# CVLAB-Unibo/Keypoint-Learning

Hardware: NVIDIA B200
Metric: points scored/sec (search+normals+features+RF+NMS) (higher is better)
Workload: dtype f32

## Files before the change

### keypoint_learning_b200/csrc/capi.cu

```cuda
#include <algorithm>
#include <cmath>
#include <cstdio>
#include <cstdlib>
#include <cstring>
#include <numeric>
#include "kpl_internal.h"

namespace kpl {
int pack_forest(const HostForestArrays& in, std::vector<PackedNode>& nodes, std::vector<int32_t>& roots, int& max_depth, int& max_var, std::string& err);
cudaError_t launch_all_flags(kpl_ctx* c, int64_t n);
}
using namespace kpl;

#define KPL_CUDA(call)                                                                              \
    do {                                                                                            \
        cudaError_t e__ = (call);                                                                   \
        if (e__ != cudaSuccess) {                                                                   \
            char b__[512];                                                                          \
            snprintf(b__, sizeof b__, "%s:%d: %s -> %s", __FILE__, __LINE__, #call, cudaGetErrorString(e__)); \
            ctx->err = b__;                                                                         \
            return e__ == cudaErrorMemoryAllocation ? KPL_E_NOMEM : KPL_E_CUDA;                     \
        }                                                                                           \
    } while (0)

static int fail(kpl_ctx* ctx, int code, const std::string& msg)
{
    ctx->err = msg;
    return code;
}

static float dec_float(uint32_t u)
{
    uint32_t b = (u & 0x80000000u) ? (u & 0x7FFFFFFFu) : ~u;
    float f;
    memcpy(&f, &b, 4);
    return f;
}

template <typename T>
static void release(DevBuf<T>& b) { if (b.p) cudaFree(b.p); b.p = nullptr; b.cap = 0; }

extern "C" {

const char* kpl_version(void) { return "kpl-b200 0.1 (sm_100a)"; }

int kpl_device_count(void)
{
    int count = 0, usable = 0;
    if (cudaGetDeviceCount(&count) != cudaSuccess) { (void)cudaGetLastError(); return 0; }
    for (int d = 0; d < count; ++d) {
        cudaDeviceProp prop;
        if (cudaGetDeviceProperties(&prop, d) == cudaSuccess && prop.major == 10) usable++;
    }
    return usable;
}

int kpl_params_default(kpl_params* p)
{
    if (!p) return KPL_E_INVALID;
    memset(p, 0, sizeof *p);
    p->radius_features = 20.f;
    p->radius_nms = 4.f;
    p->threshold = (double)0.85f;
    p->n_annulus = 5;
    p->n_bins = 10;
    p->non_maxima = 1;
    p->draws_remove = 0;
    p->draws_threshold = 0.f;
    p->normals_mode = KPL_NORMALS_KNN;
    p->k_normals = 10;
    p->flip_normals = 0;
    p->cells_per_radius = 4;
    p->grid_forced = 0;
    p->slab_interior_lo = p->slab_interior_hi = 0;
    p->slab_guard_cells = 0;
    p->slab_owned_lo = p->slab_owned_hi = 0;
    p->uniform_sampling_centre = 0;
    p->eigen32_normalize = 0;
    p->report_fragile = 0;
    return KPL_OK;
}

int kpl_create(int device, kpl_ctx** out)
{
    if (!out) return KPL_E_INVALID;
    *out = nullptr;
    int count = 0;
    if (cudaGetDeviceCount(&count) != cudaSuccess || count <= 0 || device < 0 || device >= count) return KPL_E_CUDA;
    cudaDeviceProp prop;
    if (cudaGetDeviceProperties(&prop, device) != cudaSuccess) return KPL_E_CUDA;
    if (prop.major != 10) return KPL_E_CUDA;
    if (cudaSetDevice(device) != cudaSuccess) return KPL_E_CUDA;
    kpl_ctx* ctx = new (std::nothrow) kpl_ctx();
    if (!ctx) return KPL_E_NOMEM;
    ctx->device = device;
    kpl_params_default(&ctx->params);
    memset(&ctx->timings, 0, sizeof ctx->timings);
    memset(&ctx->stats, 0, sizeof ctx->stats);
    bool ok = cudaStreamCreateWithFlags(&ctx->own_stream, cudaStreamNonBlocking) == cudaSuccess;
    ctx->stream = ctx->own_stream;
    for (int i = 0; ok && i < 8; ++i) ok = cudaEventCreate(&ctx->ev[i]) == cudaSuccess;
    ok = ok && cudaMalloc((void**)&ctx->d_bbox, 8 * sizeof(uint32_t)) == cudaSuccess;
    ok = ok && ensure(ctx->counters, kpl_ctx::NCOUNTERS) == cudaSuccess;
    if (!ok) { kpl_destroy(ctx); return KPL_E_CUDA; }
    *out = ctx;
    return KPL_OK;
}

void kpl_destroy(kpl_ctx* ctx)
{
    if (!ctx) return;
    cudaSetDevice(ctx->device);
    if (ctx->own_stream) cudaStreamSynchronize(ctx->own_stream);
    release(ctx->in_xyz); release(ctx->in_nrm); release(ctx->in_role); release(ctx->s_role);
    release(ctx->key_a); release(ctx->key_b); release(ctx->idx_a); release(ctx->idx_b); release(ctx->cub_tmp);
    release(ctx->row_warps_n); release(ctx->row_offset_n); release(ctx->fragile); release(ctx->views); release(ctx->layer_view);
    release(ctx->view_offsets); release(ctx->qlist);
    release(ctx->cell_start); release(ctx->work_n); release(ctx->ckey_a); release(ctx->ckey_b); release(ctx->qorder_a); release(ctx->qorder_all); release(ctx->warp_starts_n); release(ctx->qorder_role); release(ctx->warp_starts_role);
    release(ctx->warp_order); release(ctx->s_pos); release(ctx->s_nrm); release(ctx->feat);
    release(ctx->s_score); release(ctx->score); release(ctx->flag); release(ctx->s_state); release(ctx->kp_idx);
    release(ctx->scratch_f); release(ctx->scratch_i); release(ctx->counters);
    if (ctx->d_bbox) cudaFree(ctx->d_bbox);
    if (ctx->forest.d_nodes) cudaFree(ctx->forest.d_nodes);
    if (ctx->forest.d_roots) cudaFree(ctx->forest.d_roots);
    for (int i = 0; i < 8; ++i) if (ctx->ev[i]) cudaEventDestroy(ctx->ev[i]);
    if (ctx->own_stream) cudaStreamDestroy(ctx->own_stream);
    delete ctx;
}

const char* kpl_last_error(const kpl_ctx* ctx) { return ctx ? ctx->err.c_str() : "null context"; }

int kpl_set_stream(kpl_ctx* ctx, void* s)
{
    if (!ctx) return KPL_E_INVALID;
    ctx->stream = s ? (cudaStream_t)s : ctx->own_stream;
    return KPL_OK;
}

int kpl_set_keep_intermediates(kpl_ctx* ctx, int on)
{
    if (!ctx) return KPL_E_INVALID;
    ctx->keep_intermediates = on != 0;
    return KPL_OK;
}

int kpl_set_params(kpl_ctx* ctx, const kpl_params* p)
{
    if (!ctx || !p) return KPL_E_INVALID;
    if (!(p->radius_features > 0.f) || !std::isfinite(p->radius_features)) return fail(ctx, KPL_E_INVALID, "radius_features must be > 0");
    if (p->radius_nms < 0.f || !std::isfinite(p->radius_nms)) return fail(ctx, KPL_E_INVALID, "radius_nms must be >= 0");
    if (p->n_annulus < 1 || p->n_bins < 1 || (int64_t)p->n_annulus * p->n_bins > 1022) return fail(ctx, KPL_E_INVALID, "annuli*bins must be in [1,1022]");
    if (p->normals_mode < 0 || p->normals_mode > 2) return fail(ctx, KPL_E_INVALID, "bad normals_mode");
    if (p->k_normals < 1 || p->k_normals > 64) return fail(ctx, KPL_E_INVALID, "k_normals must be in [1,64]");
    if (p->cells_per_radius < 1 || p->cells_per_radius > 16) return fail(ctx, KPL_E_INVALID, "cells_per_radius must be in [1,16]");
    ctx->params = *p;
    return KPL_OK;
}

int kpl_get_params(const kpl_ctx* ctx, kpl_params* p)
{
    if (!ctx || !p) return KPL_E_INVALID;
    *p = ctx->params;
    return KPL_OK;
}

static int install_forest(kpl_ctx* ctx, const HostForestArrays& H)
{
    std::vector<PackedNode> nodes;
    std::vector<int32_t> roots;
    int max_depth = 0, max_var = -1;
    std::string err;
    int rc = pack_forest(H, nodes, roots, max_depth, max_var, err);
    if (rc) return fail(ctx, rc, err);
    if (roots.empty()) return fail(ctx, KPL_E_FOREST, "forest has no trees");
    KPL_CUDA(cudaSetDevice(ctx->device));
    Forest& F = ctx->forest;
    if (F.d_nodes) cudaFree(F.d_nodes);
    if (F.d_roots) cudaFree(F.d_roots);
    F.d_nodes = nullptr; F.d_roots = nullptr; F.ntrees = 0;
    KPL_CUDA(cudaMalloc((void**)&F.d_nodes, nodes.size() * sizeof(PackedNode)));
    KPL_CUDA(cudaMalloc((void**)&F.d_roots, roots.size() * sizeof(int32_t)));
    KPL_CUDA(cudaMemcpy(F.d_nodes, nodes.data(), nodes.size() * sizeof(PackedNode), cudaMemcpyHostToDevice));
    KPL_CUDA(cudaMemcpy(F.d_roots, roots.data(), roots.size() * sizeof(int32_t), cudaMemcpyHostToDevice));
    F.ntrees = (int32_t)roots.size(); F.nnodes = (int32_t)H.var.size(); F.var_count = H.var_count; F.max_depth = max_depth; F.max_var = max_var;
    F.roots = roots;
    return KPL_OK;
}

int kpl_load_forest(kpl_ctx* ctx, const char* path)
{
    if (!ctx || !path) return KPL_E_INVALID;
    HostForestArrays H;
    std::string err;
    int rc = parse_forest_yaml(path, H, err);
    if (rc) return fail(ctx, rc, err);
    return install_forest(ctx, H);
}

int kpl_set_forest(kpl_ctx* ctx, int32_t ntrees, int32_t nnodes, const int32_t* roots, const int32_t* var, const float* thr,
                   const int32_t* left, const int32_t* right, const float* value, int32_t var_count)
{
    if (!ctx || ntrees < 1 || nnodes < 1 || !roots || !var || !thr || !left || !right || !value) return KPL_E_INVALID;
    HostForestArrays H;
    H.roots.assign(roots, roots + ntrees); H.var.assign(var, var + nnodes); H.thr.assign(thr, thr + nnodes);
    H.left.assign(left, left + nnodes); H.right.assign(right, right + nnodes); H.value.assign(value, value + nnodes);
    H.var_count = var_count;
    return install_forest(ctx, H);
}

int kpl_forest_info(const kpl_ctx* ctx, int32_t* ntrees, int32_t* nnodes, int32_t* var_count, int32_t* max_depth)
{
    if (!ctx) return KPL_E_INVALID;
    if (ntrees) *ntrees = ctx->forest.ntrees;
    if (nnodes) *nnodes = ctx->forest.nnodes;
    if (var_count) *var_count = ctx->forest.var_count;
    if (max_depth) *max_depth = ctx->forest.max_depth;
    return KPL_OK;
}

}

static const double CELL_PAD = 1.0 + 9.5367431640625e-07;
static const double REACH_PAD = 1.0 + 4.76837158203125e-07;

double kpl::canonical_cell(const kpl_params& P) { return (double)P.radius_features * CELL_PAD / (double)P.cells_per_radius; }
int32_t kpl::grid_dim(double lo, double hi, double cell) { return (int32_t)std::min(2147483000.0, std::floor((hi - lo) / cell) + 1.0); }
int kpl::grid_reach(double radius, double cell) { return (int)std::floor(radius * REACH_PAD / cell) + 1; }

static void clear_batch(GridDesc& g)
{
    g.views = nullptr; g.layer_view = nullptr; g.view_offsets = nullptr; g.nviews = 0;
    g.interior_lo = g.interior_hi = 0; g.guard_cells = 0;
    g.forced = 0;
}

static int finish_grid(kpl_ctx* ctx, int64_t n)
{
    GridDesc& g = ctx->grid;
    const kpl_params& P = ctx->params;
    double ncells = 1.0;
    for (int a = 0; a < 3; ++a) {
        if (g.dim[a] < 1) return fail(ctx, KPL_E_GRID, "bad grid dimensions");
        ncells *= (double)g.dim[a];
    }
    if (ncells > 2147483646.0) return fail(ctx, KPL_E_GRID, "uniform grid would exceed 2^31-2 cells: cloud too sparse for radius_features/cells_per_radius");
    g.ncells = (int64_t)ncells;
    g.reach_feat = grid_reach(P.radius_features, g.cell);
    g.reach_nms = grid_reach(P.radius_nms, g.cell);
    ctx->stats.grid_cells = g.ncells;
    for (int a = 0; a < 3; ++a) { ctx->stats.grid_dims[a] = g.dim[a]; ctx->stats.grid_origin[a] = g.org[a]; }
    ctx->stats.grid_cell = g.cell;
    ctx->last_n = n;
    return KPL_OK;
}

int kpl::prepare_grid(kpl_ctx* ctx, const float4* d_xyz, const float4* d_nrm, const uint8_t* d_role, int64_t n, const ForcedGrid* forced, double cell_override)
{
    GridDesc& g = ctx->grid;
    clear_batch(g);
    g.cell = cell_override > 0.0 ? cell_override : canonical_cell(ctx->params);
    if (forced) {
        KPL_CUDA(launch_bbox_init(ctx));
        for (int a = 0; a < 3; ++a) { g.org[a] = forced->origin[a]; g.dim[a] = forced->dims[a]; g.off[a] = forced->offset[a]; }
        g.interior_lo = forced->interior_lo; g.interior_hi = forced->interior_hi; g.guard_cells = forced->guard_cells;
        g.forced = 1;
    } else {
        KPL_CUDA(launch_bbox(ctx, d_xyz, n, ctx->d_bbox));
        uint32_t hb[8];
        KPL_CUDA(cudaMemcpyAsync(hb, ctx->d_bbox, sizeof hb, cudaMemcpyDeviceToHost, ctx->stream));
        KPL_CUDA(cudaStreamSynchronize(ctx->stream));
        ctx->syncs++;
        if (hb[6]) return fail(ctx, KPL_E_NONFINITE, "input cloud holds non-finite points");
        for (int a = 0; a < 3; ++a) {
            const double lo = (double)dec_float(hb[a]), hi = (double)dec_float(hb[3 + a]);
            g.off[a] = 0; g.org[a] = lo;
            g.dim[a] = grid_dim(lo, hi, g.cell);
        }
    }
    int rc = finish_grid(ctx, n);
    if (rc) return rc;
    ctx->cur_xyz = d_xyz;
    ctx->cur_nrm = d_nrm;
    KPL_CUDA(build_grid(ctx, d_xyz, d_nrm, d_role, n));
    return KPL_OK;
}

static int prepare_params_grid(kpl_ctx* ctx, const float4* d_xyz, const float4* d_nrm, const uint8_t* d_role, int64_t n)
{
    const kpl_params& P = ctx->params;
    if (!P.grid_forced) return prepare_grid(ctx, d_xyz, d_nrm, d_role, n, nullptr);
    ForcedGrid f;
    for (int a = 0; a < 3; ++a) { f.origin[a] = P.grid_origin[a]; f.dims[a] = P.grid_dims[a]; f.offset[a] = P.grid_offset[a]; }
    f.interior_lo = P.slab_interior_lo; f.interior_hi = P.slab_interior_hi; f.guard_cells = P.slab_guard_cells;
    return prepare_grid(ctx, d_xyz, d_nrm, d_role, n, &f);
}

static int prepare_grid_batch(kpl_ctx* ctx, const float4* d_xyz, const float4* d_nrm, int64_t n, const int64_t* h_offsets, int nviews)
{
    const kpl_params& P = ctx->params;
    GridDesc& g = ctx->grid;
    clear_batch(g);
    g.cell = canonical_cell(P);
    KPL_CUDA(ensure(ctx->view_offsets, (size_t)nviews + 1));
    KPL_CUDA(ensure(ctx->views, (size_t)nviews));
    KPL_CUDA(ensure(ctx->scratch_i, (size_t)nviews * 8 + 16));
    KPL_CUDA(cudaMemcpyAsync(ctx->view_offsets.p, h_offsets, ((size_t)nviews + 1) * sizeof(int64_t), cudaMemcpyHostToDevice, ctx->stream));
    KPL_CUDA(launch_bbox_init(ctx));
    uint32_t* d_boxes = (uint32_t*)ctx->scratch_i.p;
    KPL_CUDA(launch_bbox_views(ctx, d_xyz, n, ctx->view_offsets.p, nviews, d_boxes));
    std::vector<uint32_t> hb((size_t)nviews * 8);
    KPL_CUDA(cudaMemcpyAsync(hb.data(), d_boxes, hb.size() * sizeof(uint32_t), cudaMemcpyDeviceToHost, ctx->stream));
    KPL_CUDA(cudaStreamSynchronize(ctx->stream));
    ctx->syncs++;
    const int pad = std::max(std::max(grid_reach(P.radius_features, g.cell), grid_reach(P.radius_nms, g.cell)), 1);
    std::vector<ViewDesc> hv((size_t)nviews);
    int64_t z = 0;
    int dimx = 1, dimy = 1;
    for (int v = 0; v < nviews; ++v) {
        const uint32_t* b = hb.data() + (size_t)v * 8;
        if (b[6]) return fail(ctx, KPL_E_NONFINITE, "a view of the batch holds non-finite points");
        int d[3];
        for (int a = 0; a < 3; ++a) {
            const double lo = (double)dec_float(b[a]), hi = (double)dec_float(b[3 + a]);
            hv[(size_t)v].org[a] = lo;
            d[a] = grid_dim(lo, hi, g.cell);
        }
        dimx = std::max(dimx, d[0]); dimy = std::max(dimy, d[1]);
        hv[(size_t)v].zoff = (int32_t)z; hv[(size_t)v].dimz = d[2];
        z += (int64_t)d[2] + pad;
        if (z > 2147483000ll) return fail(ctx, KPL_E_GRID, "the stacked grid of the batch exceeds 2^31 layers");
    }
    g.dim[0] = dimx; g.dim[1] = dimy; g.dim[2] = (int32_t)(z - pad);
    for (int a = 0; a < 3; ++a) { g.off[a] = 0; g.org[a] = hv[0].org[a]; }
    int rc = finish_grid(ctx, n);
    if (rc) return rc;
    std::vector<int32_t> layer((size_t)g.dim[2], -1);
    for (int v = 0; v < nviews; ++v)
        for (int l = 0; l < hv[(size_t)v].dimz; ++l) layer[(size_t)hv[(size_t)v].zoff + l] = v;
    KPL_CUDA(ensure(ctx->layer_view, layer.size()));
    KPL_CUDA(cudaMemcpyAsync(ctx->views.p, hv.data(), hv.size() * sizeof(ViewDesc), cudaMemcpyHostToDevice, ctx->stream));
    KPL_CUDA(cudaMemcpyAsync(ctx->layer_view.p, layer.data(), layer.size() * sizeof(int32_t), cudaMemcpyHostToDevice, ctx->stream));
    KPL_CUDA(cudaStreamSynchronize(ctx->stream));
    ctx->syncs++;
    g.views = ctx->views.p; g.layer_view = ctx->layer_view.p; g.view_offsets = ctx->view_offsets.p; g.nviews = nviews;
    ctx->cur_xyz = d_xyz;
    ctx->cur_nrm = d_nrm;
    KPL_CUDA(build_grid(ctx, d_xyz, d_nrm, nullptr, n));
    return KPL_OK;
}

static int prepare_lists(kpl_ctx* ctx, bool normals_given, bool want_features, bool use_role)
{
    const kpl_params& P = ctx->params;
    int span_n = -1;
    bool curve_normals = false;
    if (!normals_given) {
        if (P.normals_mode == KPL_NORMALS_KNN) curve_normals = normals_knn_uses_work_list(P);
        else if (P.normals_mode == KPL_NORMALS_RADIUS) span_n = P.cells_per_radius;
    }
    const int64_t slots = 148 * 28;
    const int64_t longest_first_below = ctx->last_n * 32 < (int64_t)120e6 ? 24 * slots : 0;
    KPL_CUDA(build_lists(ctx, ctx->last_n, span_n, curve_normals, want_features, use_role, longest_first_below));
    return KPL_OK;
}

static int prepare_normals(kpl_ctx* ctx, bool given, int64_t n)
{
    const kpl_params& P = ctx->params;
    if (!given) {
        if (P.normals_mode == KPL_NORMALS_KNN) KPL_CUDA(launch_normals_knn(ctx, n));
        else if (P.normals_mode == KPL_NORMALS_RADIUS) KPL_CUDA(launch_normals_radius(ctx, n));
        else return fail(ctx, KPL_E_SIZE_MISMATCH, "normals_mode is GIVEN but no normals were passed");
        if (P.flip_normals) KPL_CUDA(launch_flip_normals(ctx, n));
    }
    ctx->last_has_normals = true;
    return KPL_OK;
}

void kpl::detect_reset(kpl_ctx* ctx)
{
    (void)cudaGetLastError();
    ctx->launches = 0;
    ctx->syncs = 0;
    ctx->err.clear();
    ctx->last_has_normals = ctx->last_has_features = ctx->last_has_fragile = false;
    memset(&ctx->timings, 0, sizeof ctx->timings);
    memset(&ctx->stats, 0, sizeof ctx->stats);
    ctx->stats.n_views = 1;
}

namespace kpl {

int detect_check(kpl_ctx* ctx, int64_t n, bool with_role)
{
    const kpl_params& P = ctx->params;
    if (n < 0 || n > 2147483000ll) return fail(ctx, KPL_E_INVALID, "point count out of range");
    if (ctx->forest.ntrees < 1) return fail(ctx, KPL_E_FOREST, "no forest loaded");
    if (P.draws_remove && P.non_maxima && with_role)
        return fail(ctx, KPL_E_UNSUPPORTED, "draws-remove NMS walks the whole cloud in index order (hpp:233-250): not available with a role array; use the kpl_shard_* entry points");
    const int F = P.n_annulus * P.n_bins;
    if (ctx->forest.var_count > 0 && ctx->forest.var_count != F) return fail(ctx, KPL_E_VARCOUNT, "annuli*bins does not match the forest's var_count");
    if (ctx->forest.max_var >= F) return fail(ctx, KPL_E_VARCOUNT, "the forest splits on a variable index >= annuli*bins");
    return KPL_OK;
}

int detect_score_phase(kpl_ctx* ctx, bool normals_given, bool use_role, int64_t n)
{
    const kpl_params& P = ctx->params;
    const int F = P.n_annulus * P.n_bins;
    int rc = prepare_lists(ctx, normals_given, true, use_role);
    if (rc) return rc;
    KPL_CUDA(cudaEventRecord(ctx->ev[1], ctx->stream));
    rc = prepare_normals(ctx, normals_given, n);
    if (rc) return rc;
    KPL_CUDA(launch_check_normals(ctx, n, use_role));
    KPL_CUDA(cudaEventRecord(ctx->ev[2], ctx->stream));
    bool fuse = true;
#ifdef KPL_EXPERIMENTS
    fuse = getenv("KPL_NO_FUSE") == nullptr;
#endif
    const bool rows = ctx->keep_intermediates || !fuse;
    KPL_CUDA(launch_features(ctx, n, use_role, fuse, rows));
    ctx->last_has_features = rows; ctx->last_F = F;
// ... 527 lines not shown
```

### keypoint_learning_b200/csrc/kpl_internal.h

```cpp
#pragma once
#include <cuda_runtime.h>
#include <stdint.h>
#include <string>
#include <vector>
#include "../../include/kpl.h"

namespace kpl {

struct ViewDesc {
    double org[3];
    int32_t zoff, dimz;
};
struct GridDesc {
    double org[3];
    double cell;
    int32_t dim[3];
    int32_t off[3];
    int32_t reach_feat;
    int32_t reach_nms;
    int64_t ncells;
    const ViewDesc* views;
    const int32_t* layer_view;
    const int64_t* view_offsets;
    int32_t nviews;
    int32_t interior_lo, interior_hi;
    int32_t guard_cells;
    int32_t forced;
};

struct ForcedGrid {
    double origin[3];
    int32_t dims[3], offset[3];
    int32_t interior_lo, interior_hi, guard_cells;
};

struct __align__(8) PackedNode {
    float thr;
    uint32_t packed;
};
static constexpr uint32_t KPL_LEAF_VAR = 1023u;

struct Forest {
    int32_t ntrees = 0, nnodes = 0, var_count = 0, max_depth = 0;
    int32_t max_var = -1;
    std::vector<int32_t> roots;
    PackedNode* d_nodes = nullptr;
    int32_t* d_roots = nullptr;
};

template <typename T>
struct DevBuf {
    T* p = nullptr;
    size_t cap = 0;
};

struct HostForestArrays {
    std::vector<int32_t> roots, var, left, right;
    std::vector<float> thr, value;
    int32_t var_count = 0;
};

int parse_forest_yaml(const char* path, HostForestArrays& out, std::string& err);

}

struct kpl_ctx {
    int device = 0;
    cudaStream_t own_stream = nullptr;
    cudaStream_t stream = nullptr;
    kpl_params params;
    kpl::Forest forest;
    kpl::GridDesc grid;
    kpl_timings timings;
    kpl_stats stats;
    std::string err;
    int launches = 0;

    kpl::DevBuf<float4> in_xyz, in_nrm;
    kpl::DevBuf<uint8_t> in_role, s_role;
    kpl::DevBuf<uint32_t> key_a, key_b, idx_a, idx_b;
    kpl::DevBuf<uint8_t> cub_tmp;
    kpl::DevBuf<int32_t> cell_start;
    kpl::DevBuf<int32_t> row_warps_n, row_offset_n;
    int nwarps_norm = 0, nwarps_feat = 0;
    kpl::DevBuf<int2> work_n;
    kpl::DevBuf<uint64_t> ckey_a, ckey_b;
    kpl::DevBuf<int32_t> qorder_a, qorder_all, warp_starts_n, qorder_role, warp_starts_role;
    const int32_t* qorder_f = nullptr;
    const int32_t* warp_starts_f = nullptr;
    kpl::DevBuf<uint32_t> warp_order;
    bool have_warp_order = false;
    kpl::DevBuf<float4> s_pos, s_nrm;
    kpl::DevBuf<float> feat;
    kpl::DevBuf<float> s_score, score;
    kpl::DevBuf<uint8_t> flag;
    kpl::DevBuf<uint8_t> fragile;
    kpl::DevBuf<kpl::ViewDesc> views;
    kpl::DevBuf<int32_t> layer_view;
    kpl::DevBuf<int64_t> view_offsets;
    kpl::DevBuf<int32_t> qlist;
    kpl::DevBuf<uint8_t> s_state;
    kpl::DevBuf<int32_t> kp_idx;
    kpl::DevBuf<float> scratch_f;
    kpl::DevBuf<int32_t> scratch_i;
    kpl::DevBuf<unsigned long long> counters;
    static constexpr int NCOUNTERS = 16;
    int syncs = 0;
    const float4* cur_xyz = nullptr;
    const float4* cur_nrm = nullptr;
    float* d_bbox = nullptr;
    int64_t last_n = 0;
    int last_F = 0;
    bool last_has_normals = false, last_has_features = false, last_has_fragile = false;
    bool fast_math = false;
    bool keep_intermediates = false;
    cudaEvent_t ev[8] = {nullptr, nullptr, nullptr, nullptr, nullptr, nullptr, nullptr, nullptr};
};

namespace kpl {

cudaError_t launch_bbox(kpl_ctx* c, const float4* xyz, int64_t n, float* d_bbox );
cudaError_t build_grid(kpl_ctx* c, const float4* xyz, const float4* nrm_or_null, const uint8_t* role_or_null, int64_t n);
cudaError_t launch_normals_knn(kpl_ctx* c, int64_t n);
cudaError_t launch_normals_radius(kpl_ctx* c, int64_t n);
cudaError_t launch_flip_normals(kpl_ctx* c, int64_t n);
cudaError_t launch_check_normals(kpl_ctx* c, int64_t n, bool use_role);
bool normals_knn_uses_work_list(const kpl_params& P);
cudaError_t launch_bbox_init(kpl_ctx* c);
cudaError_t launch_gather_keypoints(kpl_ctx* c, const float4* d_xyz, const int32_t* d_kp_idx, int64_t nkp, float4* d_out);
cudaError_t launch_normals_integral_image(kpl_ctx* c, const float4* d_xyz, int W, int H, float smoothing_size, float4* d_out);
cudaError_t build_lists(kpl_ctx* c, int64_t n, int span_n, bool curve_normals, bool want_features, bool use_role, int64_t longest_first_below);
cudaError_t launch_count_occupied_cells(kpl_ctx* c, int64_t n, unsigned long long* d_out);
cudaError_t build_query_list(kpl_ctx* c, int64_t n, const int32_t* d_indices, int64_t m);
cudaError_t launch_scatter_rows(kpl_ctx* c, const float* d_rows, int64_t m, int width, float* d_out);
cudaError_t launch_view_ranges(kpl_ctx* c, int64_t n, int32_t* d_kp_idx, const int64_t* d_view_offsets, int nviews, int64_t* d_kp_offsets);
cudaError_t launch_bbox_views(kpl_ctx* c, const float4* xyz, int64_t n, const int64_t* d_view_offsets, int nviews, uint32_t* d_bbox);
cudaError_t launch_features(kpl_ctx* c, int64_t n, bool use_role, bool fuse_forest, bool store_rows, const int32_t* d_qlist = nullptr, int64_t m_list = 0);
#ifdef KPL_EXPERIMENTS
cudaError_t launch_forest(kpl_ctx* c, int64_t n, bool use_role);
#endif
cudaError_t launch_nms(kpl_ctx* c, int64_t n, bool use_role);
cudaError_t launch_nms_draws(kpl_ctx* c, int64_t n, bool use_role);
cudaError_t launch_nms_draws_classify(kpl_ctx* c, int64_t n, bool use_role);
cudaError_t launch_nms_draws_round(kpl_ctx* c, int64_t n, bool use_role, const int32_t* gidx);
cudaError_t launch_nms_draws_flags(kpl_ctx* c, int64_t n, bool use_role);
inline int nms_round_cap(int64_t n) { return (int)(n < (1 << 20) ? n : (1 << 20)); }
cudaError_t launch_compact(kpl_ctx* c, int64_t n, int32_t* d_kp_idx_out);

cudaError_t uniform_sample(kpl_ctx* c, const float4* xyz, int64_t n, float leaf, const float mn[3], const float mx[3],
                           int32_t* d_idx_out, std::string& err);
cudaError_t launch_nearest(kpl_ctx* c, const float4* d_queries, int64_t m, int32_t* d_idx, float* d_d2);
cudaError_t launch_radius_stats(kpl_ctx* c, int64_t n, double radius, int32_t* d_counts, unsigned long long* d_hash);
cudaError_t launch_radius_lists(kpl_ctx* c, int64_t n, double radius, const int32_t* d_queries, int64_t m,
                                const int64_t* d_offsets, int32_t* d_indices);
cudaError_t launch_unsort_rows(kpl_ctx* c, const float* d_sorted_rows, int64_t n, int width, float* d_out_orig_order);
cudaError_t launch_unsort_normals(kpl_ctx* c, int64_t n, float4* d_out_orig_order);

double canonical_cell(const kpl_params& P);
int32_t grid_dim(double lo, double hi, double cell);
int grid_reach(double radius, double cell);

void detect_reset(kpl_ctx* ctx);
int detect_check(kpl_ctx* ctx, int64_t n, bool with_role);
int detect_begin(kpl_ctx* ctx);
int prepare_grid(kpl_ctx* ctx, const float4* d_xyz, const float4* d_nrm, const uint8_t* d_role, int64_t n, const ForcedGrid* forced, double cell_override = 0.0);
int detect_score_phase(kpl_ctx* ctx, bool normals_given, bool use_role, int64_t n);
int detect_nms_phase(kpl_ctx* ctx, bool use_role, int64_t n, int32_t* d_kp_out);
int detect_finish(kpl_ctx* ctx, int64_t n, int64_t* n_kp_out);

template <typename T>
cudaError_t ensure(DevBuf<T>& b, size_t n)
{
    if (n <= b.cap) return cudaSuccess;
    if (b.p) cudaFree(b.p);
    b.p = nullptr; b.cap = 0;
    size_t want = n + n / 8 + 64;
    cudaError_t e = cudaMalloc((void**)&b.p, want * sizeof(T));
    if (e == cudaSuccess) b.cap = want;
    return e;
}

}
```

### keypoint_learning_b200/csrc/nms.cu

```cuda
#include <algorithm>
#include "kpl_internal.h"
#include "kpl_math.cuh"

namespace kpl {

__device__ __forceinline__ void key_to_cell_n(uint32_t key, int dimx, int dimy, int& cx, int& cy, int& cz)
{
    uint32_t t = key / (uint32_t)dimx;
    cx = (int)(key - t * (uint32_t)dimx);
    cz = (int)(t / (uint32_t)dimy);
    cy = (int)(t - (uint32_t)cz * (uint32_t)dimy);
}

__global__ void __launch_bounds__(128)
nms_kernel(const float4* __restrict__ s_pos, const float* __restrict__ s_score, const uint32_t* __restrict__ skey,
           const int32_t* __restrict__ cell_start, const uint8_t* __restrict__ s_role, int dimx, int dimy, int dimz,
           int n, float rn2, int reach, double th, uint8_t* __restrict__ flag, unsigned long long* __restrict__ counters)
{
    const int i = blockIdx.x * blockDim.x + threadIdx.x;
    bool above = false, near = false;
    if (i < n) {
        const float4 p = __ldg(s_pos + i);
        const uint32_t orig = __float_as_uint(p.w);
        const float my = __ldg(s_score + i);
        const bool owned = !s_role || ((s_role[i] & 3) == 3);
        above = owned && isfinite(my) && !((double)my < th);
        near = owned && isfinite(my) && fabs((double)my - th) <= 1e-5;
        bool is_max = above;
        if (above) {
            int cx, cy, cz;
            key_to_cell_n(__ldg(skey + i), dimx, dimy, cx, cy, cz);
            const int z0 = max(cz - reach, 0), z1 = min(cz + reach, dimz - 1);
            const int y0 = max(cy - reach, 0), y1 = min(cy + reach, dimy - 1);
            const int x0 = max(cx - reach, 0), x1 = min(cx + reach, dimx - 1);
            for (int z = z0; z <= z1 && is_max; ++z)
                for (int y = y0; y <= y1 && is_max; ++y) {
                    const int64_t base = ((int64_t)z * dimy + y) * dimx;
                    const int s = __ldg(cell_start + base + x0), e = __ldg(cell_start + base + x1 + 1);
                    for (int j = s; j < e; ++j) {
                        const float4 c = __ldg(s_pos + j);
                        if (dist2(p.x, p.y, p.z, c.x, c.y, c.z) < rn2 && my < __ldg(s_score + j)) { is_max = false; break; }
                    }
                }
        }
        flag[orig] = is_max ? 1 : 0;
    }
    unsigned m = __ballot_sync(0xFFFFFFFFu, above);
    if ((threadIdx.x & 31) == 0 && m) atomicAdd(counters + 2, (unsigned long long)__popc(m));
    m = __ballot_sync(0xFFFFFFFFu, near);
    if ((threadIdx.x & 31) == 0 && m) atomicAdd(counters + 7, (unsigned long long)__popc(m));
}

cudaError_t launch_nms(kpl_ctx* c, int64_t n, bool use_role)
{
    const kpl_params& U = c->params;
    cudaError_t e;
    if ((e = ensure(c->flag, n))) return e;
    const double rn = (double)U.radius_nms;
    nms_kernel<<<(unsigned)((n + 127) / 128), 128, 0, c->stream>>>(c->s_pos.p, c->s_score.p, c->key_b.p, c->cell_start.p,
                                                                   use_role ? c->s_role.p : nullptr,
                                                                   c->grid.dim[0], c->grid.dim[1], c->grid.dim[2], (int)n,
                                                                   (float)(rn * rn), c->grid.reach_nms, U.threshold, c->flag.p, c->counters.p);
    c->launches++;
    return cudaGetLastError();
}

__device__ __forceinline__ float draw_distance(const float4& p, const float4& c)
{
    const float dx = __fsub_rn(p.x, c.x), dy = __fsub_rn(p.y, c.y), dz = __fsub_rn(p.z, c.z);
    return __fsqrt_rn(__fadd_rn(__fmul_rn(dx, dx), __fadd_rn(__fmul_rn(dy, dy), __fmul_rn(dz, dz))));
}

template <int PASS>
__global__ void __launch_bounds__(128)
nms_draws_kernel(const float4* __restrict__ s_pos, const float* __restrict__ s_score, const uint32_t* __restrict__ skey,
                 const int32_t* __restrict__ cell_start, const uint8_t* __restrict__ s_role, int dimx, int dimy, int dimz,
                 int n, float rn2, int reach, double th, float draws_thr, const int32_t* __restrict__ gidx,
                 uint8_t* __restrict__ s_state, unsigned long long* __restrict__ counters)
{
    const int i = blockIdx.x * blockDim.x + threadIdx.x;
    bool above = false, near = false;
    if (i < n) {
        const float4 p = __ldg(s_pos + i);
        const uint32_t orig = __float_as_uint(p.w);
        const float my = __ldg(s_score + i);
        const bool owned = !s_role || ((s_role[i] & 3) == 3);
        if (PASS == 0) {
            above = owned && isfinite(my) && !((double)my < th);
            near = owned && isfinite(my) && fabs((double)my - th) <= 1e-5;
        }
        const bool work = PASS == 0 ? above : (owned && s_state[i] == 2);
        if (work) {
            int cx, cy, cz;
            key_to_cell_n(__ldg(skey + i), dimx, dimy, cx, cy, cz);
            const int z0 = max(cz - reach, 0), z1 = min(cz + reach, dimz - 1);
            const int y0 = max(cy - reach, 0), y1 = min(cy + reach, dimy - 1);
            const int x0 = max(cx - reach, 0), x1 = min(cx + reach, dimx - 1);
            bool is_max = true, has_draw = false, close_draw = false;
            bool lower_active = false, lower_undecided = false;
            const uint32_t my_order = PASS == 1 && gidx ? (uint32_t)__ldg(gidx + orig) : orig;
            for (int z = z0; z <= z1 && is_max; ++z)
                for (int y = y0; y <= y1 && is_max; ++y) {
                    const int64_t base = ((int64_t)z * dimy + y) * dimx;
                    const int s = __ldg(cell_start + base + x0), e = __ldg(cell_start + base + x1 + 1);
                    for (int j = s; j < e; ++j) {
                        const float4 c = __ldg(s_pos + j);
                        if (!(dist2(p.x, p.y, p.z, c.x, c.y, c.z) < rn2)) continue;
                        const float sj = __ldg(s_score + j);
                        if (PASS == 0) {
                            if (my < sj) { is_max = false; break; }
                            if (my == sj && j != i) {
                                has_draw = true;
                                if (draw_distance(p, c) < draws_thr) close_draw = true;
                            }
                        } else if (my == sj && (gidx ? (uint32_t)__ldg(gidx + __float_as_uint(c.w)) : __float_as_uint(c.w)) < my_order &&
                                   draw_distance(p, c) < draws_thr) {
                            const uint8_t st = s_state[j];
                            if (st == 1) lower_active = true;
                            else if (st == 2) lower_undecided = true;
                        }
                    }
                }
            if (PASS == 0) s_state[i] = !is_max ? 0 : (!has_draw ? 1 : (close_draw ? 2 : 0));
            else if (lower_active) s_state[i] = 3;
            else if (!lower_undecided) s_state[i] = 1;
            else atomicAdd(counters + 6, 1ull);
        } else if (PASS == 0) s_state[i] = 0;
    }
    if (PASS == 0) {
        unsigned m = __ballot_sync(0xFFFFFFFFu, above);
        if ((threadIdx.x & 31) == 0 && m) atomicAdd(counters + 2, (unsigned long long)__popc(m));
        m = __ballot_sync(0xFFFFFFFFu, near);
        if ((threadIdx.x & 31) == 0 && m) atomicAdd(counters + 7, (unsigned long long)__popc(m));
    }
}

__global__ void __launch_bounds__(256) state_to_flag_kernel(const float4* __restrict__ s_pos, const uint8_t* __restrict__ s_role,
                                                            const uint8_t* __restrict__ s_state, int n, uint8_t* __restrict__ flag)
{
    const int i = blockIdx.x * blockDim.x + threadIdx.x;
    if (i < n) flag[__float_as_uint(__ldg(&s_pos[i].w))] = s_state[i] == 1 && (!s_role || (s_role[i] & 3) == 3) ? 1 : 0;
}

cudaError_t launch_nms_draws_classify(kpl_ctx* c, int64_t n, bool use_role)
{
    const kpl_params& U = c->params;
    cudaError_t e;
    if ((e = ensure(c->flag, n)) || (e = ensure(c->s_state, n))) return e;
    const double rn = (double)U.radius_nms;
    nms_draws_kernel<0><<<(unsigned)((n + 127) / 128), 128, 0, c->stream>>>(c->s_pos.p, c->s_score.p, c->key_b.p, c->cell_start.p,
                                                                              use_role ? c->s_role.p : nullptr, c->grid.dim[0], c->grid.dim[1],
                                                                              c->grid.dim[2], (int)n, (float)(rn * rn), c->grid.reach_nms,
                                                                              U.threshold, U.draws_threshold, nullptr, c->s_state.p, c->counters.p);
    c->launches++;
    return cudaGetLastError();
}

cudaError_t launch_nms_draws_round(kpl_ctx* c, int64_t n, bool use_role, const int32_t* gidx)
{
    const kpl_params& U = c->params;
    cudaError_t e;
    if ((e = cudaMemsetAsync(c->counters.p + 6, 0, sizeof(unsigned long long), c->stream))) return e;
    const double rn = (double)U.radius_nms;
    nms_draws_kernel<1><<<(unsigned)((n + 127) / 128), 128, 0, c->stream>>>(c->s_pos.p, c->s_score.p, c->key_b.p, c->cell_start.p,
                                                                              use_role ? c->s_role.p : nullptr, c->grid.dim[0], c->grid.dim[1],
                                                                              c->grid.dim[2], (int)n, (float)(rn * rn), c->grid.reach_nms,
                                                                              U.threshold, U.draws_threshold, gidx, c->s_state.p, c->counters.p);
    c->launches++;
    c->stats.nms_rounds++;
    return cudaGetLastError();
}

cudaError_t launch_nms_draws_flags(kpl_ctx* c, int64_t n, bool use_role)
{
    state_to_flag_kernel<<<(unsigned)((n + 255) / 256), 256, 0, c->stream>>>(c->s_pos.p, use_role ? c->s_role.p : nullptr, c->s_state.p,
                                                                            (int)n, c->flag.p);
    c->launches++;
    return cudaGetLastError();
}

cudaError_t launch_nms_draws(kpl_ctx* c, int64_t n, bool use_role)
{
    cudaError_t e;
    if ((e = launch_nms_draws_classify(c, n, use_role))) return e;
    for (int round = 0; round < nms_round_cap(n); ++round) {
        if ((e = launch_nms_draws_round(c, n, use_role, nullptr))) return e;
        unsigned long long undecided = 0;
        if ((e = cudaMemcpyAsync(&undecided, c->counters.p + 6, sizeof undecided, cudaMemcpyDeviceToHost, c->stream))) return e;
        if ((e = cudaStreamSynchronize(c->stream))) return e;
        c->syncs++;
        if (undecided == 0) break;
    }
    return launch_nms_draws_flags(c, n, use_role);
}

__global__ void __launch_bounds__(256) all_flags_kernel(const float* __restrict__ score, int64_t n, uint8_t* __restrict__ flag)
{
    int64_t i = blockIdx.x * (int64_t)blockDim.x + threadIdx.x;
    if (i < n) flag[i] = isnan(score[i]) ? 0 : 1;
}
cudaError_t launch_all_flags(kpl_ctx* c, int64_t n)
{
    cudaError_t e;
    if ((e = ensure(c->flag, n))) return e;
    all_flags_kernel<<<(unsigned)((n + 255) / 256), 256, 0, c->stream>>>(c->score.p, n, c->flag.p);
    c->launches++;
    return cudaGetLastError();
}

static constexpr unsigned long long HASH_MUL = 0x9E3779B97F4A7C15ull;

template <bool LISTS>
__global__ void __launch_bounds__(128)
radius_kernel(const float4* __restrict__ s_pos, const uint32_t* __restrict__ skey, const int32_t* __restrict__ cell_start,
              const int32_t* __restrict__ inv_or_queries, int dimx, int dimy, int dimz, int n, int64_t m, float r2, int reach,
              int32_t* __restrict__ counts, unsigned long long* __restrict__ hash,
              const int64_t* __restrict__ offsets, int32_t* __restrict__ indices)
{
    const int64_t t = blockIdx.x * (int64_t)blockDim.x + threadIdx.x;
    if (t >= m) return;
    const int i = LISTS ? inv_or_queries[t] : (int)t;
    const float4 p = __ldg(s_pos + i);
    int cx, cy, cz;
    key_to_cell_n(__ldg(skey + i), dimx, dimy, cx, cy, cz);
    const int z0 = max(cz - reach, 0), z1 = min(cz + reach, dimz - 1);
    const int y0 = max(cy - reach, 0), y1 = min(cy + reach, dimy - 1);
    const int x0 = max(cx - reach, 0), x1 = min(cx + reach, dimx - 1);
    int cnt = 0;
    unsigned long long h = 0;
    int64_t w = LISTS ? offsets[t] : 0;
    for (int z = z0; z <= z1; ++z)
        for (int y = y0; y <= y1; ++y) {
            const int64_t base = ((int64_t)z * dimy + y) * dimx;
            const int s = __ldg(cell_start + base + x0), e = __ldg(cell_start + base + x1 + 1);
            for (int j = s; j < e; ++j) {
                const float4 c = __ldg(s_pos + j);
                if (dist2(p.x, p.y, p.z, c.x, c.y, c.z) < r2) {
                    const uint32_t oj = __float_as_uint(c.w);
                    if (LISTS) indices[w++] = (int32_t)oj;
                    cnt++;
                    h += ((unsigned long long)oj + 1ull) * HASH_MUL;
                }
            }
        }
    if (!LISTS) {
        const uint32_t orig = __float_as_uint(p.w);
        if (counts) counts[orig] = cnt;
        if (hash) hash[orig] = h;
    }
}

__global__ void __launch_bounds__(128)
nearest_kernel(const float4* __restrict__ s_pos, const int32_t* __restrict__ cell_start, GridDesc g, const float4* __restrict__ queries,
               int64_t m, int32_t* __restrict__ idx_out, float* __restrict__ d2_out)
{
    const int64_t t = blockIdx.x * (int64_t)blockDim.x + threadIdx.x;
    if (t >= m) return;
    const float4 q = __ldg(queries + t);
    const float v[3] = {q.x, q.y, q.z};
    int c[3];
#pragma unroll
    for (int a = 0; a < 3; ++a) {
        double f = floor(__ddiv_rn(__dsub_rn((double)v[a], g.org[a]), g.cell)) - (double)g.off[a];
        f = fmin(fmax(f, 0.0), (double)(g.dim[a] - 1));
        c[a] = isfinite(v[a]) ? (int)f : 0;
    }
    float best = CUDART_INF_F;
    uint32_t bidx = 0xFFFFFFFFu;
    auto scan = [&](int z, int y, int x0, int x1) {
        x0 = max(x0, 0); x1 = min(x1, g.dim[0] - 1);
        if (z < 0 || z >= g.dim[2] || y < 0 || y >= g.dim[1] || x0 > x1) return;
        const int64_t base = ((int64_t)z * g.dim[1] + y) * g.dim[0];
        const int s = __ldg(cell_start + base + x0), e = __ldg(cell_start + base + x1 + 1);
        for (int j = s; j < e; ++j) {
            const float4 p = __ldg(s_pos + j);
            const float d2 = dist2(q.x, q.y, q.z, p.x, p.y, p.z);
            const uint32_t oi = __float_as_uint(p.w);
            if (d2 < best || (d2 == best && oi < bidx)) { best = d2; bidx = oi; }
        }
    };
    const int maxdim = max(g.dim[0], max(g.dim[1], g.dim[2]));
    for (int R = 0; R <= maxdim; ++R) {
        for (int z = c[2] - R; z <= c[2] + R; ++z)
            for (int y = c[1] - R; y <= c[1] + R; ++y) {
                if (abs(z - c[2]) == R || abs(y - c[1]) == R) scan(z, y, c[0] - R, c[0] + R);
                else { scan(z, y, c[0] - R, c[0] - R); if (R > 0) scan(z, y, c[0] + R, c[0] + R); }
            }
        if (bidx != 0xFFFFFFFFu) {
            double guard = (double)R * g.cell;
            guard = guard * guard * (1.0 - 1e-6);
            if ((double)best < guard) break;
        }
    }
    idx_out[t] = (int32_t)bidx;
    if (d2_out) d2_out[t] = best;
}

cudaError_t launch_nearest(kpl_ctx* c, const float4* d_queries, int64_t m, int32_t* d_idx, float* d_d2)
{
    if (m == 0) return cudaSuccess;
    nearest_kernel<<<(unsigned)((m + 127) / 128), 128, 0, c->stream>>>(c->s_pos.p, c->cell_start.p, c->grid, d_queries, m, d_idx, d_d2);
    c->launches++;
    return cudaGetLastError();
}

static int reach_for(const GridDesc& g, double radius)
{
    return (int)floor(radius * (1.0 + 4.76837158203125e-07) / g.cell) + 1;
}

cudaError_t launch_radius_stats(kpl_ctx* c, int64_t n, double radius, int32_t* d_counts, unsigned long long* d_hash)
{
    radius_kernel<false><<<(unsigned)((n + 127) / 128), 128, 0, c->stream>>>(
        c->s_pos.p, c->key_b.p, c->cell_start.p, nullptr, c->grid.dim[0], c->grid.dim[1], c->grid.dim[2], (int)n, n,
        (float)(radius * radius), reach_for(c->grid, radius), d_counts, d_hash, nullptr, nullptr);
    c->launches++;
    return cudaGetLastError();
}

cudaError_t launch_radius_lists(kpl_ctx* c, int64_t n, double radius, const int32_t* d_queries, int64_t m,
                                const int64_t* d_offsets, int32_t* d_indices)
{
    if (m == 0) return cudaSuccess;
    radius_kernel<true><<<(unsigned)((m + 127) / 128), 128, 0, c->stream>>>(
        c->s_pos.p, c->key_b.p, c->cell_start.p, d_queries, c->grid.dim[0], c->grid.dim[1], c->grid.dim[2], (int)n, m,
        (float)(radius * radius), reach_for(c->grid, radius), nullptr, nullptr, d_offsets, d_indices);
    c->launches++;
    return cudaGetLastError();
}

}
```

Before: 64.25 million.

## Compact above-threshold points and run warp-cooperative NMS with shared-memory tiles

NMS now runs in stages. A select kernel flags owned points above the threshold, and CUB stream compaction builds a list of those candidates. A persistent warp-cooperative kernel then processes them in dynamically fetched chunks. Inside each warp, candidates that share a cell row are grouped and check neighbour cells together through a shared-memory tile and packed dist2 math, so no work is spent on sub-threshold threads and warp divergence is lower. The cost is extra launches, a memset of the flag array, and the reuse of counter slots for the chunk counter and candidate count, which could collide with other uses.

```diff
diff --git a/keypoint_learning_b200/csrc/capi.cu b/keypoint_learning_b200/csrc/capi.cu
--- a/keypoint_learning_b200/csrc/capi.cu
+++ b/keypoint_learning_b200/csrc/capi.cu
@@ -118,7 +118,7 @@
     release(ctx->view_offsets); release(ctx->qlist);
     release(ctx->cell_start); release(ctx->work_n); release(ctx->ckey_a); release(ctx->ckey_b); release(ctx->qorder_a); release(ctx->qorder_all); release(ctx->warp_starts_n); release(ctx->qorder_role); release(ctx->warp_starts_role);
     release(ctx->warp_order); release(ctx->s_pos); release(ctx->s_nrm); release(ctx->feat);
-    release(ctx->s_score); release(ctx->score); release(ctx->flag); release(ctx->s_state); release(ctx->kp_idx);
+    release(ctx->s_score); release(ctx->score); release(ctx->flag); release(ctx->s_state); release(ctx->nms_list); release(ctx->kp_idx);
     release(ctx->scratch_f); release(ctx->scratch_i); release(ctx->counters);
     if (ctx->d_bbox) cudaFree(ctx->d_bbox);
     if (ctx->forest.d_nodes) cudaFree(ctx->forest.d_nodes);
diff --git a/keypoint_learning_b200/csrc/kpl_internal.h b/keypoint_learning_b200/csrc/kpl_internal.h
--- a/keypoint_learning_b200/csrc/kpl_internal.h
+++ b/keypoint_learning_b200/csrc/kpl_internal.h
@@ -100,6 +100,7 @@
     kpl::DevBuf<int64_t> view_offsets;
     kpl::DevBuf<int32_t> qlist;
     kpl::DevBuf<uint8_t> s_state;
+    kpl::DevBuf<int32_t> nms_list;
     kpl::DevBuf<int32_t> kp_idx;
     kpl::DevBuf<float> scratch_f;
     kpl::DevBuf<int32_t> scratch_i;
diff --git a/keypoint_learning_b200/csrc/nms.cu b/keypoint_learning_b200/csrc/nms.cu
--- a/keypoint_learning_b200/csrc/nms.cu
+++ b/keypoint_learning_b200/csrc/nms.cu
@@ -1,4 +1,6 @@
 #include <algorithm>
+#include <cub/device/device_select.cuh>
+#include <thrust/iterator/counting_iterator.h>
 #include "kpl_internal.h"
 #include "kpl_math.cuh"
 
@@ -12,38 +14,18 @@
     cy = (int)(t - (uint32_t)cz * (uint32_t)dimy);
 }
 
-__global__ void __launch_bounds__(128)
-nms_kernel(const float4* __restrict__ s_pos, const float* __restrict__ s_score, const uint32_t* __restrict__ skey,
-           const int32_t* __restrict__ cell_start, const uint8_t* __restrict__ s_role, int dimx, int dimy, int dimz,
-           int n, float rn2, int reach, double th, uint8_t* __restrict__ flag, unsigned long long* __restrict__ counters)
+__global__ void __launch_bounds__(256)
+nms_select_kernel(const float* __restrict__ s_score, const uint8_t* __restrict__ s_role, int n, double th,
+                  uint8_t* __restrict__ above_out, unsigned long long* __restrict__ counters)
 {
     const int i = blockIdx.x * blockDim.x + threadIdx.x;
     bool above = false, near = false;
     if (i < n) {
-        const float4 p = __ldg(s_pos + i);
-        const uint32_t orig = __float_as_uint(p.w);
         const float my = __ldg(s_score + i);
         const bool owned = !s_role || ((s_role[i] & 3) == 3);
         above = owned && isfinite(my) && !((double)my < th);
         near = owned && isfinite(my) && fabs((double)my - th) <= 1e-5;
-        bool is_max = above;
-        if (above) {
-            int cx, cy, cz;
-            key_to_cell_n(__ldg(skey + i), dimx, dimy, cx, cy, cz);
-            const int z0 = max(cz - reach, 0), z1 = min(cz + reach, dimz - 1);
-            const int y0 = max(cy - reach, 0), y1 = min(cy + reach, dimy - 1);
-            const int x0 = max(cx - reach, 0), x1 = min(cx + reach, dimx - 1);
-            for (int z = z0; z <= z1 && is_max; ++z)
-                for (int y = y0; y <= y1 && is_max; ++y) {
-                    const int64_t base = ((int64_t)z * dimy + y) * dimx;
-                    const int s = __ldg(cell_start + base + x0), e = __ldg(cell_start + base + x1 + 1);
-                    for (int j = s; j < e; ++j) {
-                        const float4 c = __ldg(s_pos + j);
-                        if (dist2(p.x, p.y, p.z, c.x, c.y, c.z) < rn2 && my < __ldg(s_score + j)) { is_max = false; break; }
-                    }
-                }
-        }
-        flag[orig] = is_max ? 1 : 0;
+        above_out[i] = above ? 1 : 0;
     }
     unsigned m = __ballot_sync(0xFFFFFFFFu, above);
     if ((threadIdx.x & 31) == 0 && m) atomicAdd(counters + 2, (unsigned long long)__popc(m));
@@ -51,17 +33,103 @@
     if ((threadIdx.x & 31) == 0 && m) atomicAdd(counters + 7, (unsigned long long)__popc(m));
 }
 
+constexpr int NMS_SPAN = 1;
+constexpr int NMS_WARPS = 4;
+__global__ void __launch_bounds__(32 * NMS_WARPS)
+nms_coop_kernel(const float4* __restrict__ s_pos, const float* __restrict__ s_score, const uint32_t* __restrict__ skey,
+                const int32_t* __restrict__ cell_start, const int32_t* __restrict__ list, const int32_t* __restrict__ d_count,
+                int* __restrict__ next_chunk, int dimx, int dimy, int dimz, float rn2, int reach, uint64_t one2, uint8_t* __restrict__ flag)
+{
+    __shared__ __align__(16) float tile[NMS_WARPS][128];
+    const int lane = threadIdx.x & 31;
+    float* sx = tile[threadIdx.x >> 5]; float* sy = sx + 32; float* sz = sx + 64; float* ss = sx + 96;
+    const int count = __ldg(d_count);
+    const int side = 2 * reach + 1, nrows = side * side, centre = reach * side + reach;
+#pragma unroll 1
+    for (;;) {
+    int chunk = 0;
+    if (lane == 0) chunk = atomicAdd(next_chunk, 1);
+    const int base_e = __shfl_sync(0xFFFFFFFFu, chunk, 0) * 32;
+    if (base_e >= count) return;
+    const bool active = base_e + lane < count;
+    const int i = active ? __ldg(list + base_e + lane) : 0;
+    float4 p = make_float4(CUDART_NAN_F, 0.f, 0.f, 0.f);
+    float my = CUDART_NAN_F;
+    int cx = 0x3FFFFFFF, cy = -1, cz = -1;
+    if (active) { p = __ldg(s_pos + i); my = __ldg(s_score + i); key_to_cell_n(__ldg(skey + i), dimx, dimy, cx, cy, cz); }
+    const uint64_t QY = pack2(p.y, p.y), QZ = pack2(p.z, p.z);
+    bool sup = false;
+    unsigned remaining = __ballot_sync(0xFFFFFFFFu, active);
+    while (remaining) {
+        const int leader = __ffs(remaining) - 1;
+        const int lx = __shfl_sync(0xFFFFFFFFu, cx, leader), ly = __shfl_sync(0xFFFFFFFFu, cy, leader), lz = __shfl_sync(0xFFFFFFFFu, cz, leader);
+        const bool member = ((remaining >> lane) & 1u) && cy == ly && cz == lz && (unsigned)(cx - lx) <= (unsigned)NMS_SPAN;
+        remaining &= ~__ballot_sync(0xFFFFFFFFu, member);
+        const int gx1 = __reduce_max_sync(0xFFFFFFFFu, member ? cx : lx);
+        const int xa = max(lx - reach, 0), xb = min(gx1 + reach, dimx - 1);
+        const float px = member ? p.x : CUDART_NAN_F;
+        const uint64_t QX = pack2(px, px);
+        bool open = true;
+#pragma unroll 1
+        for (int r = 0; r < nrows && open; ++r) {
+            const int rr = r == 0 ? centre : (r == centre ? 0 : r);
+            const int y = ly - reach + rr % side, z = lz - reach + rr / side;
+            if (y < 0 || y >= dimy || z < 0 || z >= dimz) continue;
+            const int64_t rowb = ((int64_t)z * dimy + y) * dimx;
+            const int rs = __ldg(cell_start + rowb + xa), re = __ldg(cell_start + rowb + xb + 1);
+            for (int tb = rs; tb < re && open; tb += 32) {
+                float4 c = make_float4(CUDART_NAN_F, 0.f, 0.f, 0.f);
+                float cs = CUDART_NAN_F;
+                if (tb + lane < re) { c = __ldg(s_pos + tb + lane); cs = __ldg(s_score + tb + lane); }
+                __syncwarp();
+                sx[lane] = c.x; sy[lane] = c.y; sz[lane] = c.z; ss[lane] = cs;
+                __syncwarp();
+                const int cnt = min(32, re - tb);
+                bool hit = false;
+#pragma unroll
+                for (int k0 = 0; k0 < 32; k0 += 4) {
+                    if (k0 < cnt) {
+                        const ulonglong2 X = *reinterpret_cast<const ulonglong2*>(sx + k0);
+                        const ulonglong2 Y = *reinterpret_cast<const ulonglong2*>(sy + k0);
+                        const ulonglong2 Z = *reinterpret_cast<const ulonglong2*>(sz + k0);
+                        const float4 S = *reinterpret_cast<const float4*>(ss + k0);
+                        float d0, d1, d2, d3;
+                        unpack2(dist2_x2(QX, QY, QZ, X.x, Y.x, Z.x, one2), d0, d1);
+                        unpack2(dist2_x2(QX, QY, QZ, X.y, Y.y, Z.y, one2), d2, d3);
+                        hit |= (d0 < rn2 && my < S.x) | (d1 < rn2 && my < S.y) | (d2 < rn2 && my < S.z) | (d3 < rn2 && my < S.w);
+                    }
+                }
+                sup |= member && hit;
+                open = __any_sync(0xFFFFFFFFu, member && !sup);
+            }
+        }
+    }
+    if (active && !sup) flag[__float_as_uint(p.w)] = 1;
+    }
+}
+
 cudaError_t launch_nms(kpl_ctx* c, int64_t n, bool use_role)
 {
     const kpl_params& U = c->params;
     cudaError_t e;
-    if ((e = ensure(c->flag, n))) return e;
+    if ((e = ensure(c->flag, n)) || (e = ensure(c->s_state, n)) || (e = ensure(c->nms_list, n))) return e;
+    int32_t* d_count = reinterpret_cast<int32_t*>(c->counters.p + 10);
+    int* d_next = reinterpret_cast<int*>(c->counters.p + 6);
+    thrust::counting_iterator<int32_t> it(0);
+    size_t bytes = 0;
+    cub::DeviceSelect::Flagged(nullptr, bytes, it, c->s_state.p, c->nms_list.p, d_count, (int)n, c->stream);
+    if ((e = ensure(c->cub_tmp, bytes))) return e;
+    if ((e = cudaMemsetAsync(c->flag.p, 0, (size_t)n, c->stream)) || (e = cudaMemsetAsync(d_next, 0, sizeof(int), c->stream))) return e;
     const double rn = (double)U.radius_nms;
-    nms_kernel<<<(unsigned)((n + 127) / 128), 128, 0, c->stream>>>(c->s_pos.p, c->s_score.p, c->key_b.p, c->cell_start.p,
-                                                                   use_role ? c->s_role.p : nullptr,
-                                                                   c->grid.dim[0], c->grid.dim[1], c->grid.dim[2], (int)n,
-                                                                   (float)(rn * rn), c->grid.reach_nms, U.threshold, c->flag.p, c->counters.p);
-    c->launches++;
+    nms_select_kernel<<<(unsigned)((n + 255) / 256), 256, 0, c->stream>>>(c->s_score.p, use_role ? c->s_role.p : nullptr, (int)n, U.threshold,
+                                                                        c->s_state.p, c->counters.p);
+    bytes = c->cub_tmp.cap;
+    if ((e = cub::DeviceSelect::Flagged(c->cub_tmp.p, bytes, it, c->s_state.p, c->nms_list.p, d_count, (int)n, c->stream))) return e;
+    const int64_t blocks = std::min<int64_t>((n + 32 * NMS_WARPS - 1) / (32 * NMS_WARPS), 148 * 8);
+    nms_coop_kernel<<<(unsigned)blocks, 32 * NMS_WARPS, 0, c->stream>>>(
+        c->s_pos.p, c->s_score.p, c->key_b.p, c->cell_start.p, c->nms_list.p, d_count, d_next, c->grid.dim[0], c->grid.dim[1], c->grid.dim[2],
+        (float)(rn * rn), c->grid.reach_nms, 0x3F8000003F800000ull, c->flag.p);
+    c->launches += 4;
     return cudaGetLastError();
 }
 
```

New measurement: 64.70 million (median of 6 runs). Within noise of the previous version (+0.7%).
